# facebookresearch/fast3r

Hardware: NVIDIA H100
Metric: views_per_sec (higher is better)
Workload: dtype bf16

## Files before the change

fast3r_b200/csrc/capi.cu:

```cuda
#include <cstdarg>
#include <cstdio>
#include <cstdlib>
#include <cstring>

#include "../../include/fast3r_b200.h"
#include "f3r_kernels.h"
#include "gemm_plan.h"

namespace {

thread_local char g_err[512] = "";

int fail(const char* fmt, ...) {
  va_list ap;
  va_start(ap, fmt);
  vsnprintf(g_err, sizeof(g_err), fmt, ap);
  va_end(ap);
  return 1;
}
int check(cudaError_t e, const char* what) {
  if (e == cudaSuccess) return 0;
  return fail("%s: %s", what, cudaGetErrorString(e));
}

// ... 68 lines not shown
  if (d->k % 8 || d->a_ld % 8) return fail("f3r_gemm: k=%d and a_ld=%d must be multiples of 8", d->k, d->a_ld);
  if (d->taps != 1 && d->taps != 9) return fail("f3r_gemm: taps must be 1 or 9");
  if (d->epi == F3R_EPI_FINAL && d->n != 128) return fail("f3r_gemm: FINAL epilogue needs n == 128");
  if (d->epi == F3R_EPI_CONVT && (d->ct_k <= 0 || d->ct_cout % 32 || d->n != d->ct_k * d->ct_k * d->ct_cout))
    return fail("f3r_gemm: bad CONVT geometry");
  if (d->epi == F3R_EPI_ROPE && (!d->rope_cos || !d->rope_sin || d->tok_per_img <= 0 || d->grid_w <= 0))
    return fail("f3r_gemm: bad ROPE arguments");
  if (d->epi == F3R_EPI_IDXEMB && (!d->emb_table || !d->emb_ids || d->tok_per_img < 0))
    return fail("f3r_gemm: bad IDXEMB arguments");
  if (d->f16 != 0 && d->f16 != 1) return fail("f3r_gemm: f16=%d must be 0 or 1", d->f16);

  static int dbg = -1, tma_pref = -1, ksplit_pref = -1;
  if (dbg < 0) { const char* e = getenv("F3R_GEMM_DEBUG"); dbg = e ? atoi(e) : 0; }
  if (tma_pref < 0) { const char* e = getenv("F3R_GEMM_TMA_EPI"); tma_pref = (e && e[0] == '0') ? 0 : 1; }
  if (ksplit_pref < 0) { const char* e = getenv("F3R_GEMM_KSPLIT"); ksplit_pref = (e && e[0] == '1') ? 1 : 0; }
  const f3r::GemmPlan plan = f3r::gemm_plan(*d, num_sms(), tma_pref, ksplit_pref != 1);
  const int block_n = plan.block_n;

  f3r::GemmArgs a;
  memset(&a, 0, sizeof(a));
  a.M = d->w * d->h * d->nb; a.N = d->n; a.K = d->k; a.taps = d->taps;
  a.W = d->w; a.H = d->h; a.NB = d->nb;
  a.bw = plan.bw; a.bh = plan.bh; a.bw_log2 = plan.bw_log2; a.sbx_log2 = plan.sbx_log2;
  a.tiles_x = plan.tiles_x; a.tiles_y = plan.tiles_y; a.num_m_tiles = plan.num_m_tiles;
  a.num_n_tiles = plan.num_n_tiles;
  a.tma_epi = plan.tma_epi; a.k_split = plan.k_split;
  a.debug = dbg;
  a.epi = d->epi; a.act = d->act; a.out0_f32 = d->out0_f32; a.res0_f32 = d->res0_f32;
  a.ldo = d->ldo > 0 ? d->ldo : d->n;
  a.split_col = d->split_col; a.ldo_b = d->ldo_b;
  a.tok_per_img = d->tok_per_img; a.grid_w = d->grid_w; a.rope_cols = d->rope_cols;
  a.ct_k = d->ct_k; a.ct_cout = d->ct_cout;
  a.bias = d->bias; a.res0 = d->res0; a.res1 = d->res1;
  a.out0 = d->out0; a.out0b = d->out0b; a.out1 = d->out1;
  a.rope_cos = d->rope_cos; a.rope_sin = d->rope_sin;
  a.emb_table = d->emb_table; a.emb_ids = d->emb_ids;
  a.w4 = d->w4; a.b4 = d->b4; a.pts = d->pts; a.conf = d->conf;
  if (a.split_col && (a.split_col % 32 || !a.out0b)) return fail("f3r_gemm: bad column split");

  const CUtensorMapDataType t16 = d->f16 ? CU_TENSOR_MAP_DATA_TYPE_FLOAT16 : CU_TENSOR_MAP_DATA_TYPE_BFLOAT16;
  CUtensorMap ta, tb;
  {
    const uint64_t ld = static_cast<uint64_t>(d->a_ld) * 2;
    const uint64_t dims[4] = {static_cast<uint64_t>(d->k), static_cast<uint64_t>(d->w),
                              static_cast<uint64_t>(d->h), static_cast<uint64_t>(d->nb)};
    const uint64_t str[3] = {ld, ld * d->w, ld * d->w * d->h};
    const uint32_t box[4] = {64, static_cast<uint32_t>(a.bw), static_cast<uint32_t>(a.bh), 1};
    if (make_tmap(&ta, d->a, 4, dims, str, box, t16)) return 1;
  }
  {
    const uint64_t dims[3] = {static_cast<uint64_t>(d->k), static_cast<uint64_t>(d->taps),
                              static_cast<uint64_t>(d->n)};
    const uint64_t str[2] = {static_cast<uint64_t>(d->k) * 2, static_cast<uint64_t>(d->k) * 2 * d->taps};
    const uint32_t box[3] = {64, 1, static_cast<uint32_t>(block_n)};
    if (make_tmap(&tb, d->wt, 3, dims, str, box, t16)) return 1;
  }
  CUtensorMap to0, to0b;
  memset(&to0, 0, sizeof(to0));
  memset(&to0b, 0, sizeof(to0b));
  if (a.tma_epi) {
    const uint64_t es = d->out0_f32 ? 4 : 2;
    const CUtensorMapDataType dt = d->out0_f32 ? CU_TENSOR_MAP_DATA_TYPE_FLOAT32 : t16;
    const CUtensorMapSwizzle sw = d->out0_f32 ? CU_TENSOR_MAP_SWIZZLE_128B : CU_TENSOR_MAP_SWIZZLE_64B;
    const uint32_t sbx = 1u << a.sbx_log2;
    const uint32_t box[4] = {32, sbx, 32 / sbx, 1};
    const uint64_t ncols0 = a.split_col ? a.split_col : d->n;
    {
      const uint64_t ld = static_cast<uint64_t>(a.ldo) * es;
      const uint64_t dims[4] = {ncols0, static_cast<uint64_t>(d->w), static_cast<uint64_t>(d->h),
                                static_cast<uint64_t>(d->nb)};
      const uint64_t str[3] = {ld, ld * d->w, ld * d->w * d->h};
      if (make_tmap(&to0, d->out0, 4, dims, str, box, dt, sw)) return 1;
    }
    if (a.split_col) {
      const uint64_t ld = static_cast<uint64_t>(a.ldo_b) * es;
      const uint64_t dims[4] = {static_cast<uint64_t>(d->n - a.split_col), static_cast<uint64_t>(d->w),
                                static_cast<uint64_t>(d->h), static_cast<uint64_t>(d->nb)};
      const uint64_t str[3] = {ld, ld * d->w, ld * d->w * d->h};
      if (make_tmap(&to0b, d->out0b, 4, dims, str, box, dt, sw)) return 1;
    }
  }
  return check(f3r::launch_gemm(block_n, d->f16, ta, tb, to0, to0b, a, num_sms(), static_cast<cudaStream_t>(stream)),
               "f3r_gemm");
}

static int attention_impl(const char* what, int f16, const void* q, int32_t ldq, const void* kv, int32_t ldkv,
                          int32_t kv_rows_total, int32_t kv_row0, void* out, int32_t ldo, float* lse, float* part_o,
                          float* part_lse, int32_t part_base, int32_t n_split, int32_t batch, int32_t heads, int32_t sq,
                          int32_t skv, float scale, void* stream) {
  const CUtensorMapDataType t16 = f16 ? CU_TENSOR_MAP_DATA_TYPE_FLOAT16 : CU_TENSOR_MAP_DATA_TYPE_BFLOAT16;
  if (!q || !kv) return fail("%s: null operand", what);
  if (batch <= 0 || heads <= 0 || sq <= 0 || skv <= 0) return fail("%s: bad shape", what);
  if (ldq % 8 || ldkv % 8 || ldq < heads * 64 || ldkv < 2 * heads * 64) return fail("%s: bad leading dimensions", what);
  if (kv_row0 < 0 || kv_row0 + skv > kv_rows_total) return fail("%s: key range outside the kv buffer", what);
  if (n_split < 1 || n_split > (skv + 127) / 128) return fail("%s: n_split=%d must be in [1, #key blocks]", what, n_split);
  CUtensorMap tq, tkv;
  {
    const uint64_t dims[3] = {static_cast<uint64_t>(heads) * 64, static_cast<uint64_t>(sq),
                              static_cast<uint64_t>(batch)};
    const uint64_t str[2] = {static_cast<uint64_t>(ldq) * 2, static_cast<uint64_t>(ldq) * 2 * sq};
    const uint32_t box[3] = {64, f3r::ATT_Q_TILE, 1};
    if (make_tmap(&tq, q, 3, dims, str, box, t16)) return 1;
  }
  {
    const uint64_t dims[3] = {static_cast<uint64_t>(heads) * 128, static_cast<uint64_t>(kv_row0 + skv),
                              static_cast<uint64_t>(batch)};
    const uint64_t str[2] = {static_cast<uint64_t>(ldkv) * 2, static_cast<uint64_t>(ldkv) * 2 * kv_rows_total};
// ... 549 lines not shown
```

fast3r_b200/csrc/common.cuh:

```cuda
#pragma once
#include <cuda.h>
#include <cuda_bf16.h>
#include <cuda_fp16.h>
#include <cuda_runtime.h>
#include <stdint.h>

#include <type_traits>

namespace f3r {

#define F3R_DEVICE __device__ __forceinline__

F3R_DEVICE uint32_t smem_u32(const void* p) { return static_cast<uint32_t>(__cvta_generic_to_shared(p)); }

F3R_DEVICE uint32_t lane_id() { return threadIdx.x & 31; }

F3R_DEVICE bool elect_one() {
  uint32_t pred = 0;
  asm volatile(
      "{\n\t.reg .pred P;\n\t"
      "elect.sync _|P, 0xffffffff;\n\t"
      "selp.u32 %0, 1, 0, P;\n\t}\n"
      : "=r"(pred));
  return pred != 0;
// ... 16 lines not shown
  asm volatile(
      "{\n\t.reg .pred P;\n\t"
      "mbarrier.try_wait.parity.shared::cta.b64 P, [%1], %2;\n\t"
      "selp.u32 %0, 1, 0, P;\n\t}\n"
      : "=r"(ok)
      : "r"(smem_u32(bar)), "r"(parity)
      : "memory");
  return ok != 0;
}
F3R_DEVICE void mbar_wait(uint64_t* bar, uint32_t parity) {
  while (!mbar_try_wait(bar, parity)) {
  }
}

F3R_DEVICE void mbar_wait_relaxed(uint64_t* bar, uint32_t parity) {
  while (!mbar_try_wait(bar, parity)) asm volatile("nanosleep.u32 64;");
}

F3R_DEVICE void tma_prefetch_desc(const CUtensorMap* m) {
  asm volatile("prefetch.tensormap [%0];" ::"l"(reinterpret_cast<uint64_t>(m)) : "memory");
}
F3R_DEVICE void tma_load_2d(void* dst, const CUtensorMap* m, uint64_t* bar, int c0, int c1) {
  asm volatile(
      "cp.async.bulk.tensor.2d.shared::cluster.global.mbarrier::complete_tx::bytes [%0], [%1, {%3, %4}], [%2];"
      ::"r"(smem_u32(dst)), "l"(reinterpret_cast<uint64_t>(m)), "r"(smem_u32(bar)), "r"(c0), "r"(c1)
      : "memory");
}
F3R_DEVICE void tma_load_3d(void* dst, const CUtensorMap* m, uint64_t* bar, int c0, int c1, int c2) {
  asm volatile(
      "cp.async.bulk.tensor.3d.shared::cluster.global.mbarrier::complete_tx::bytes [%0], [%1, {%3, %4, %5}], [%2];"
      ::"r"(smem_u32(dst)), "l"(reinterpret_cast<uint64_t>(m)), "r"(smem_u32(bar)), "r"(c0), "r"(c1), "r"(c2)
      : "memory");
}
F3R_DEVICE void tma_load_4d(void* dst, const CUtensorMap* m, uint64_t* bar, int c0, int c1, int c2, int c3) {
  asm volatile(
      "cp.async.bulk.tensor.4d.shared::cluster.global.mbarrier::complete_tx::bytes [%0], [%1, {%3, %4, %5, %6}], [%2];"
      ::"r"(smem_u32(dst)), "l"(reinterpret_cast<uint64_t>(m)), "r"(smem_u32(bar)), "r"(c0), "r"(c1), "r"(c2),
      "r"(c3)
      : "memory");
}

F3R_DEVICE void tma_store_4d(const CUtensorMap* m, const void* src, int c0, int c1, int c2, int c3) {
  asm volatile("cp.async.bulk.tensor.4d.global.shared::cta.bulk_group [%0, {%2, %3, %4, %5}], [%1];"
               ::"l"(reinterpret_cast<uint64_t>(m)), "r"(smem_u32(src)), "r"(c0), "r"(c1), "r"(c2), "r"(c3)
               : "memory");
}
F3R_DEVICE void tma_reduce_add_4d(const CUtensorMap* m, const void* src, int c0, int c1, int c2, int c3) {
  asm volatile("cp.reduce.async.bulk.tensor.4d.global.shared::cta.add.tile.bulk_group [%0, {%2, %3, %4, %5}], [%1];"
               ::"l"(reinterpret_cast<uint64_t>(m)), "r"(smem_u32(src)), "r"(c0), "r"(c1), "r"(c2), "r"(c3)
               : "memory");
}
F3R_DEVICE void tma_store_commit() { asm volatile("cp.async.bulk.commit_group;" ::: "memory"); }
F3R_DEVICE void tma_store_wait_read() { asm volatile("cp.async.bulk.wait_group.read 0;" ::: "memory"); }
F3R_DEVICE void tma_store_wait_all() { asm volatile("cp.async.bulk.wait_group 0;" ::: "memory"); }

F3R_DEVICE void pdl_wait() { asm volatile("griddepcontrol.wait;" ::: "memory"); }
F3R_DEVICE void pdl_launch_dependents() { asm volatile("griddepcontrol.launch_dependents;" ::: "memory"); }

F3R_DEVICE uint32_t cluster_ctarank() { uint32_t r; asm volatile("mov.u32 %0, %%cluster_ctarank;" : "=r"(r)); return r; }
F3R_DEVICE uint32_t cluster_id_x() { uint32_t r; asm volatile("mov.u32 %0, %%clusterid.x;" : "=r"(r)); return r; }
F3R_DEVICE uint32_t num_clusters_x() { uint32_t r; asm volatile("mov.u32 %0, %%nclusterid.x;" : "=r"(r)); return r; }
F3R_DEVICE void cluster_sync_all() {
  asm volatile("barrier.cluster.arrive.release.aligned;" ::: "memory");
  asm volatile("barrier.cluster.wait.acquire.aligned;" ::: "memory");
}

F3R_DEVICE uint64_t make_smem_desc_sw128(uint32_t smem_addr) {
  uint64_t d = 0;
  d |= static_cast<uint64_t>((smem_addr & 0x3FFFF) >> 4);
  d |= static_cast<uint64_t>(1) << 16;
  d |= static_cast<uint64_t>(1024 >> 4) << 32;
  d |= static_cast<uint64_t>(1) << 62;
  return d;
}
F3R_DEVICE void wgmma_fence() { asm volatile("wgmma.fence.sync.aligned;" ::: "memory"); }
F3R_DEVICE void wgmma_commit() { asm volatile("wgmma.commit_group.sync.aligned;" ::: "memory"); }
template <int kPending>
F3R_DEVICE void wgmma_wait() { asm volatile("wgmma.wait_group.sync.aligned %0;" ::"n"(kPending) : "memory"); }
template <int kN>
F3R_DEVICE void fence_regs(float (&d)[kN]) {
#pragma unroll
  for (int i = 0; i < kN; ++i) asm volatile("" : "+f"(d[i])::"memory");
}


template <typename T>
constexpr bool is_f16 = std::is_same<T, __half>::value;

#define F3R_WGMMA_SS_N128(TY) \
  asm volatile( \
      "{\n\t.reg .pred p;\n\t" \
      "setp.ne.b32 p, %66, 0;\n\t" \
      "wgmma.mma_async.sync.aligned.m64n128k16.f32." TY "." TY " {%0, %1, %2, %3, %4, %5, %6, %7, %8, %9, %10, %11, %12, %13, %14, %15, %16, %17, %18, %19, %20, %21, %22, %23, %24, %25, %26, %27, %28, %29, %30, %31, %32, %33, %34, %35, %36, %37, %38, %39, %40, %41, %42, %43, %44, %45, %46, %47, %48, %49, %50, %51, %52, %53, %54, %55, %56, %57, %58, %59, %60, %61, %62, %63}, %64, %65, p, 1, 1, 0, %67;\n\t}\n" \
      : "+f"(d[0]), "+f"(d[1]), "+f"(d[2]), "+f"(d[3]), "+f"(d[4]), "+f"(d[5]), "+f"(d[6]), "+f"(d[7]), "+f"(d[8]), "+f"(d[9]), "+f"(d[10]), "+f"(d[11]), "+f"(d[12]), "+f"(d[13]), "+f"(d[14]), "+f"(d[15]), "+f"(d[16]), "+f"(d[17]), "+f"(d[18]), "+f"(d[19]), "+f"(d[20]), "+f"(d[21]), "+f"(d[22]), "+f"(d[23]), "+f"(d[24]), "+f"(d[25]), "+f"(d[26]), "+f"(d[27]), "+f"(d[28]), "+f"(d[29]), "+f"(d[30]), "+f"(d[31]), "+f"(d[32]), "+f"(d[33]), "+f"(d[34]), "+f"(d[35]), "+f"(d[36]), "+f"(d[37]), "+f"(d[38]), "+f"(d[39]), "+f"(d[40]), "+f"(d[41]), "+f"(d[42]), "+f"(d[43]), "+f"(d[44]), "+f"(d[45]), "+f"(d[46]), "+f"(d[47]), "+f"(d[48]), "+f"(d[49]), "+f"(d[50]), "+f"(d[51]), "+f"(d[52]), "+f"(d[53]), "+f"(d[54]), "+f"(d[55]), "+f"(d[56]), "+f"(d[57]), "+f"(d[58]), "+f"(d[59]), "+f"(d[60]), "+f"(d[61]), "+f"(d[62]), "+f"(d[63]) \
      : "l"(a_desc), "l"(b_desc), "r"(accumulate), "n"(kTransB))
template <int kTransB, typename T = __nv_bfloat16>
F3R_DEVICE void wgmma_ss_n128(float (&d)[64], uint64_t a_desc, uint64_t b_desc, uint32_t accumulate) {
  if constexpr (is_f16<T>) F3R_WGMMA_SS_N128("f16");
  else F3R_WGMMA_SS_N128("bf16");
}

#define F3R_WGMMA_SS_N256(TY) \
  asm volatile( \
      "{\n\t.reg .pred p;\n\t" \
      "setp.ne.b32 p, %130, 0;\n\t" \
      "wgmma.mma_async.sync.aligned.m64n256k16.f32." TY "." TY " {%0, %1, %2, %3, %4, %5, %6, %7, %8, %9, %10, %11, %12, %13, %14, %15, %16, %17, %18, %19, %20, %21, %22, %23, %24, %25, %26, %27, %28, %29, %30, %31, %32, %33, %34, %35, %36, %37, %38, %39, %40, %41, %42, %43, %44, %45, %46, %47, %48, %49, %50, %51, %52, %53, %54, %55, %56, %57, %58, %59, %60, %61, %62, %63, %64, %65, %66, %67, %68, %69, %70, %71, %72, %73, %74, %75, %76, %77, %78, %79, %80, %81, %82, %83, %84, %85, %86, %87, %88, %89, %90, %91, %92, %93, %94, %95, %96, %97, %98, %99, %100, %101, %102, %103, %104, %105, %106, %107, %108, %109, %110, %111, %112, %113, %114, %115, %116, %117, %118, %119, %120, %121, %122, %123, %124, %125, %126, %127}, %128, %129, p, 1, 1, 0, %131;\n\t}\n" \
// ... 50 lines not shown
```

fast3r_b200/csrc/gemm.cu:

```cuda
#include "common.cuh"
#include "f3r_kernels.h"

namespace f3r {

constexpr int BLOCK_M = 128;
constexpr int BLOCK_K = 64;
constexpr int GEMM_THREADS = 384;
constexpr int XCH_STRIDE = 68;

template <int BLOCK_N>
struct GemmCfg {
  static constexpr int kStages = (BLOCK_N == 256) ? 3 : 4;
  static constexpr int kABytes = BLOCK_M * BLOCK_K * 2;
  static constexpr int kBBytes = BLOCK_N * BLOCK_K * 2;
  static constexpr int kStageBytes = kABytes + kBBytes;
  static constexpr int kXchBytes = 64 * XCH_STRIDE * 4;
  static constexpr int kSmemBytes =
      kStages * kStageBytes + 1024  + 1024  + 8 * 4096  + 2 * kXchBytes;
};

struct ResChunk {
  uint4 r0[8];
  uint2 r1[8];
};

__device__ __forceinline__ size_t out_offset(const GemmArgs& p, int m, int col0, int img, int py, int px) {
  if (p.epi == EPI_CONVT) {
    const int ij = col0 / p.ct_cout, o0 = col0 % p.ct_cout, k = p.ct_k;
    const int oy = py * k + ij / k, ox = px * k + ij % k;
    return ((static_cast<size_t>(img) * p.H * k + oy) * (p.W * k) + ox) * p.ct_cout + o0;
  }
  return static_cast<size_t>(m) * p.ldo + col0;
}

__device__ __forceinline__ void prefetch_res(const GemmArgs& p, ResChunk& rc, size_t off_row, bool ok_row, int lane) {
  if (p.res0 == nullptr && p.res1 == nullptr) return;
  const unsigned okmask = __ballot_sync(0xffffffffu, ok_row);
#pragma unroll
  for (int i = 0; i < 8; ++i) {
    const int rr = 4 * i + (lane >> 3);
    const size_t off = __shfl_sync(0xffffffffu, off_row, rr) + (lane & 7) * 4;
    if (!((okmask >> rr) & 1)) continue;
    if (p.res0 != nullptr) {
      if (p.res0_f32) rc.r0[i] = *reinterpret_cast<const uint4*>(static_cast<const float*>(p.res0) + off);
      else {
        const uint2 t = *reinterpret_cast<const uint2*>(static_cast<const uint16_t*>(p.res0) + off);
        rc.r0[i].x = t.x; rc.r0[i].y = t.y;
      }
    }
    if (p.res1 != nullptr) rc.r1[i] = *reinterpret_cast<const uint2*>(static_cast<const uint16_t*>(p.res1) + off);
  }
}

__device__ __forceinline__ void gelu_fast(float& x) {
  const float z = __fmul_rn(fabsf(x), 0.70710678118654752440f);
  const float u = fmaf(z, 0.3275911f, 1.0f);
  float t;
  asm("rcp.approx.ftz.f32 %0, %1;" : "=f"(t) : "f"(u));
  float q = fmaf(t, 1.061405429f, -1.453152027f);
  q = fmaf(q, t, 1.421413741f);
  q = fmaf(q, t, -0.284496736f);
  q = fmaf(q, t, 0.254829592f);
  q = __fmul_rn(q, t);
  const float a = __fmul_rn(__fmul_rn(z, z), -1.4426950408889634f);
  float e;
  asm("ex2.approx.ftz.f32 %0, %1;" : "=f"(e) : "f"(a));
  const float r = copysignf(fmaf(q, -e, 1.0f), x);
// ... 10 lines not shown
      v[4 * i + 0] += b.x; v[4 * i + 1] += b.y; v[4 * i + 2] += b.z; v[4 * i + 3] += b.w;
    }
  }
  if (p.epi == EPI_ROPE && col0 < p.rope_cols && row_ok) {
    const int t = m % p.tok_per_img;
    const int pos = ((col0 >> 5) & 1) ? (t % p.grid_w) : (t / p.grid_w);
    const float4* c4 = reinterpret_cast<const float4*>(p.rope_cos + pos * 16);
    const float4* s4 = reinterpret_cast<const float4*>(p.rope_sin + pos * 16);
#pragma unroll
    for (int i = 0; i < 4; ++i) {
      float4 c = __ldg(c4 + i), s = __ldg(s4 + i);
      float cc[4] = {c.x, c.y, c.z, c.w}, ss[4] = {s.x, s.y, s.z, s.w};
#pragma unroll
      for (int e = 0; e < 4; ++e) {
        const int j = 4 * i + e;
        const float a = v[j], b = v[j + 16];
        v[j] = a * cc[e] - b * ss[e];
        v[j + 16] = b * cc[e] + a * ss[e];
      }
    }
  }
  if (p.epi == EPI_IDXEMB && row_ok) {
    const int id = __ldg(p.emb_ids + (p.tok_per_img > 0 ? m / p.tok_per_img : m));
    const float4* e4 = reinterpret_cast<const float4*>(p.emb_table + static_cast<size_t>(id) * p.N + col0);
#pragma unroll
    for (int i = 0; i < 8; ++i) {
      float4 e = __ldg(e4 + i);
      v[4 * i + 0] += e.x; v[4 * i + 1] += e.y; v[4 * i + 2] += e.z; v[4 * i + 3] += e.w;
    }
  }
  if (p.epi == EPI_FINAL) {
    if (row_ok) {
#pragma unroll
      for (int o = 0; o < 4; ++o) {
        const float4* w = reinterpret_cast<const float4*>(w4s + o * p.N + col0);
        float acc = fin[o];
#pragma unroll
        for (int i = 0; i < 8; ++i) {
          const float4 ww = w[i];
          acc = fmaf(fmaxf(v[4 * i + 0], 0.f), ww.x, acc);
          acc = fmaf(fmaxf(v[4 * i + 1], 0.f), ww.y, acc);
          acc = fmaf(fmaxf(v[4 * i + 2], 0.f), ww.z, acc);
          acc = fmaf(fmaxf(v[4 * i + 3], 0.f), ww.w, acc);
        }
        fin[o] = acc;
      }
    }
    return false;
  }
  return true;
}

template <typename T>
__device__ __forceinline__ void epilogue_store(const GemmArgs& p, const float (&v)[32], const ResChunk& rc, uint8_t* stage,
                                               int lane, int m, int col0, size_t off_row, bool ok_row) {
  using H = Half16<T>;
#pragma unroll
  for (int j = 0; j < 8; ++j)
    *reinterpret_cast<float4*>(stage + lane * 128 + ((j ^ (lane & 7)) << 4)) =
        make_float4(v[4 * j], v[4 * j + 1], v[4 * j + 2], v[4 * j + 3]);
  __syncwarp();
  const unsigned okmask = __ballot_sync(0xffffffffu, ok_row);
  const int cj = lane & 7;
  const bool to_b = p.split_col > 0 && col0 >= p.split_col;
#pragma unroll
  for (int i = 0; i < 8; ++i) {
    const int rr = 4 * i + (lane >> 3);
    const size_t off = __shfl_sync(0xffffffffu, off_row, rr) + cj * 4;
    const int mrow = __shfl_sync(0xffffffffu, m, rr);
    if (!((okmask >> rr) & 1)) continue;
    const float4 a = *reinterpret_cast<const float4*>(stage + rr * 128 + ((cj ^ (rr & 7)) << 4));
    float x0 = a.x, x1 = a.y, x2 = a.z, x3 = a.w;
    if (p.res0 != nullptr) {
      if (p.res0_f32) {
        x0 += __uint_as_float(rc.r0[i].x); x1 += __uint_as_float(rc.r0[i].y);
        x2 += __uint_as_float(rc.r0[i].z); x3 += __uint_as_float(rc.r0[i].w);
      } else {
        x0 += H::lo(rc.r0[i].x); x1 += H::hi(rc.r0[i].x); x2 += H::lo(rc.r0[i].y); x3 += H::hi(rc.r0[i].y);
      }
    }
    if (p.res1 != nullptr) {
      x0 += H::lo(rc.r1[i].x); x1 += H::hi(rc.r1[i].x); x2 += H::lo(rc.r1[i].y); x3 += H::hi(rc.r1[i].y);
    }
    if (p.out1 != nullptr) {
      uint2 o;
      o.x = H::pack(fmaxf(x0, 0.f), fmaxf(x1, 0.f));
      o.y = H::pack(fmaxf(x2, 0.f), fmaxf(x3, 0.f));
      *reinterpret_cast<uint2*>(static_cast<T*>(p.out1) + off) = o;
    }
    if (p.out0 == nullptr) continue;
    if (p.act == ACT_RELU) {
      x0 = fmaxf(x0, 0.f); x1 = fmaxf(x1, 0.f); x2 = fmaxf(x2, 0.f); x3 = fmaxf(x3, 0.f);
    } else if (p.act == ACT_GELU) {
      gelu_fast(x0); gelu_fast(x1); gelu_fast(x2); gelu_fast(x3);
    }
    void* base = p.out0;
    size_t o = off;
    if (to_b) {
      base = p.out0b;
      o = static_cast<size_t>(mrow) * p.ldo_b + (col0 - p.split_col) + cj * 4;
    }
    if (p.out0_f32) {
      *reinterpret_cast<float4*>(static_cast<float*>(base) + o) = make_float4(x0, x1, x2, x3);
    } else {
      uint2 q;
      q.x = H::pack(x0, x1);
      q.y = H::pack(x2, x3);
      *reinterpret_cast<uint2*>(static_cast<T*>(base) + o) = q;
    }
  }
  __syncwarp();
}

template <typename T>
__device__ __forceinline__ void epilogue_tma(const GemmArgs& p, float (&v)[32], uint8_t* stage, int lane,
                                             const CUtensorMap* map, bool reduce, int c_col, int c_x, int c_y, int c_img) {
  if (p.act == ACT_RELU) {
#pragma unroll
    for (int i = 0; i < 32; ++i) v[i] = fmaxf(v[i], 0.f);
  } else if (p.act == ACT_GELU) {
#pragma unroll
    for (int i = 0; i < 32; ++i) gelu_fast(v[i]);
  }
  if (lane == 0) tma_store_wait_read();
  __syncwarp();
  if (p.out0_f32) {
#pragma unroll
    for (int j = 0; j < 8; ++j)
      *reinterpret_cast<float4*>(stage + lane * 128 + ((j ^ (lane & 7)) << 4)) =
          make_float4(v[4 * j], v[4 * j + 1], v[4 * j + 2], v[4 * j + 3]);
  } else {
#pragma unroll
    for (int j = 0; j < 4; ++j) {
      uint4 q;
      q.x = Half16<T>::pack(v[8 * j + 0], v[8 * j + 1]);
      q.y = Half16<T>::pack(v[8 * j + 2], v[8 * j + 3]);
      q.z = Half16<T>::pack(v[8 * j + 4], v[8 * j + 5]);
      q.w = Half16<T>::pack(v[8 * j + 6], v[8 * j + 7]);
      *reinterpret_cast<uint4*>(stage + lane * 64 + ((j ^ ((lane >> 1) & 3)) << 4)) = q;
    }
  }
  fence_proxy_async_smem();
  __syncwarp();
  if (lane == 0) {
    if (reduce) tma_reduce_add_4d(map, stage, c_col, c_x, c_y, c_img);
    else tma_store_4d(map, stage, c_col, c_x, c_y, c_img);
    tma_store_commit();
  }
}

template <int BLOCK_N, typename T>
__global__ void __launch_bounds__(GEMM_THREADS, 1)
gemm_kernel(const __grid_constant__ CUtensorMap tmap_a, const __grid_constant__ CUtensorMap tmap_b,
            const __grid_constant__ CUtensorMap tmap_o0, const __grid_constant__ CUtensorMap tmap_o0b,
            const __grid_constant__ GemmArgs p) {
  using Cfg = GemmCfg<BLOCK_N>;
  extern __shared__ uint8_t smem_raw[];
  uint8_t* smem = reinterpret_cast<uint8_t*>((reinterpret_cast<uintptr_t>(smem_raw) + 1023) & ~uintptr_t(1023));
  uint8_t* smem_a = smem;
  uint8_t* smem_b = smem + Cfg::kStages * Cfg::kABytes;
  uint64_t* bars = reinterpret_cast<uint64_t*>(smem + Cfg::kStages * Cfg::kStageBytes);
  uint64_t* full_bar = bars;
  uint64_t* empty_bar = bars + Cfg::kStages;
  uint8_t* stage_base = smem + Cfg::kStages * Cfg::kStageBytes + 1024;
  float* fin_smem = reinterpret_cast<float*>(stage_base);
  float* w4_smem = reinterpret_cast<float*>(stage_base + 4096);
  float* xch_base = reinterpret_cast<float*>(stage_base + 8 * 4096);

  const int warp = threadIdx.x >> 5;
  const int lane = threadIdx.x & 31;

  if (threadIdx.x == 0) {
    tma_prefetch_desc(&tmap_a);
    tma_prefetch_desc(&tmap_b);
    for (int s = 0; s < Cfg::kStages; ++s) { mbar_init(&full_bar[s], 1); mbar_init(&empty_bar[s], 2); }
    fence_barrier_init();
  }
  if (p.epi == EPI_FINAL)
    for (int i = threadIdx.x; i < 4 * p.N; i += GEMM_THREADS) w4_smem[i] = __ldg(p.w4 + i);
  __syncthreads();
  pdl_wait();
  pdl_launch_dependents();

  const int num_out_tiles = p.num_m_tiles * p.num_n_tiles;
  const int num_tiles = num_out_tiles * p.k_split;
  const int k_chunks = (p.K + BLOCK_K - 1) / BLOCK_K;
  const int k_iters = p.taps * k_chunks;

  if (warp < 4) {
    asm volatile("setmaxnreg.dec.sync.aligned.u32 40;");
    if (warp == 0 && lane == 0) {
      int stage = 0; uint32_t phase = 0;
      for (int item = blockIdx.x; item < num_tiles; item += gridDim.x) {
        const int tile = item % num_out_tiles, ks = item / num_out_tiles;
        const int it0 = ks * k_iters / p.k_split, it1 = (ks + 1) * k_iters / p.k_split;
        const int mt = tile / p.num_n_tiles, nt = tile % p.num_n_tiles;
        const int tx = mt % p.tiles_x, ty = (mt / p.tiles_x) % p.tiles_y, img = mt / (p.tiles_x * p.tiles_y);
        const int x0 = tx * p.bw, y0 = ty * p.bh, n0 = nt * BLOCK_N;
        for (int it = it0; it < it1; ++it) {
          const int tap = it / k_chunks, kc = it % k_chunks;
          int dy = 0, dx = 0;
          if (p.taps == 9) { dy = tap / 3 - 1; dx = tap % 3 - 1; }
          mbar_wait_relaxed(&empty_bar[stage], phase ^ 1);
          mbar_arrive_expect_tx(&full_bar[stage], Cfg::kStageBytes);
          tma_load_4d(smem_a + stage * Cfg::kABytes, &tmap_a, &full_bar[stage], kc * BLOCK_K, x0 + dx, y0 + dy, img);
          tma_load_3d(smem_b + stage * Cfg::kBBytes, &tmap_b, &full_bar[stage], kc * BLOCK_K, tap, n0);
          if (++stage == Cfg::kStages) { stage = 0; phase ^= 1; }
        }
      }
    }
  } else {
    asm volatile("setmaxnreg.inc.sync.aligned.u32 232;");
    const int cg = (warp - 4) >> 2;
    const int wg_warp = warp & 3;
    const int wg_tid = threadIdx.x & 127;
    const int half = wg_warp >> 1;
    const int r_loc = (wg_warp & 1) * 32 + lane;
    const int r = cg * 64 + r_loc;
    float* xch = xch_base + cg * 64 * XCH_STRIDE;
    uint8_t* stage_buf = stage_base + (warp - 4) * 4096;
    const int bar_id = 1 + cg;
    constexpr int kAcc = BLOCK_N / 2;
    int stage = 0; uint32_t phase = 0;
    for (int item = blockIdx.x; item < num_tiles; item += gridDim.x) {
      const int tile = item % num_out_tiles, ks = item / num_out_tiles;
      const int it0 = ks * k_iters / p.k_split, it1 = (ks + 1) * k_iters / p.k_split;
      const bool add_bias = ks == 0;
      float acc[kAcc];
#pragma unroll
      for (int i = 0; i < kAcc; ++i) acc[i] = 0.f;
      int prev = -1;
      for (int it = it0; it < it1; ++it) {
        mbar_wait(&full_bar[stage], phase);
        const uint64_t a_desc = make_smem_desc_sw128(smem_u32(smem_a + stage * Cfg::kABytes + cg * 64 * 128));
        const uint64_t b_desc = make_smem_desc_sw128(smem_u32(smem_b + stage * Cfg::kBBytes));
        fence_regs(acc);
        wgmma_fence();
#pragma unroll
        for (int k = 0; k < BLOCK_K / 16; ++k) {
          if constexpr (BLOCK_N == 256) wgmma_ss_n256<0, T>(acc, a_desc + 2 * k, b_desc + 2 * k, 1u);
          else wgmma_ss_n128<0, T>(acc, a_desc + 2 * k, b_desc + 2 * k, 1u);
        }
        wgmma_commit();
        wgmma_wait<1>();
        fence_regs(acc);
        if (prev >= 0 && wg_tid == 0) mbar_arrive(&empty_bar[prev]);
        prev = stage;
        if (++stage == Cfg::kStages) { stage = 0; phase ^= 1; }
      }
      wgmma_wait<0>();
      fence_regs(acc);
      if (prev >= 0 && wg_tid == 0) mbar_arrive(&empty_bar[prev]);

      const int mt = tile / p.num_n_tiles, nt = tile % p.num_n_tiles;
      const int tx = mt % p.tiles_x, ty = (mt / p.tiles_x) % p.tiles_y, img = mt / (p.tiles_x * p.tiles_y);
      const int px = tx * p.bw + r % p.bw, py = ty * p.bh + r / p.bw;
      const bool row_ok = (px < p.W) && (py < p.H) && (mt < p.num_m_tiles);
      const int m = (img * p.H + py) * p.W + px;
      const int n_valid = min(BLOCK_N / 32, (p.N - nt * BLOCK_N + 31) / 32);
      float fin[4] = {0.f, 0.f, 0.f, 0.f};
#pragma unroll
      for (int cp = 0; cp < BLOCK_N / 64; ++cp) {
        asm volatile("bar.sync %0, 128;" ::"r"(bar_id) : "memory");
        {
          const int fr = wg_warp * 16 + (lane >> 2), fc = 2 * (lane & 3);
#pragma unroll
          for (int j = 0; j < 8; ++j) {
            const int jj = cp * 8 + j;
            *reinterpret_cast<float2*>(xch + fr * XCH_STRIDE + 8 * j + fc) = make_float2(acc[4 * jj], acc[4 * jj + 1]);
            *reinterpret_cast<float2*>(xch + (fr + 8) * XCH_STRIDE + 8 * j + fc) =
                make_float2(acc[4 * jj + 2], acc[4 * jj + 3]);
          }
        }
        asm volatile("bar.sync %0, 128;" ::"r"(bar_id) : "memory");
        const int c = 2 * cp + half;
        if (c >= n_valid) continue;
        const int col0 = nt * BLOCK_N + c * 32;
        float v[32];
#pragma unroll
        for (int i = 0; i < 8; ++i) {
          const float4 t = *reinterpret_cast<const float4*>(xch + r_loc * XCH_STRIDE + half * 32 + 4 * i);
          v[4 * i] = t.x; v[4 * i + 1] = t.y; v[4 * i + 2] = t.z; v[4 * i + 3] = t.w;
        }
        if (epilogue_rows(p, v, m, col0, row_ok, fin, add_bias, w4_smem) && !(p.debug & 1)) {
          if (p.tma_epi) {
            const bool to_b = p.split_col > 0 && col0 >= p.split_col;
            const int r0 = cg * 64 + (wg_warp & 1) * 32;
            epilogue_tma<T>(p, v, stage_buf, lane, to_b ? &tmap_o0b : &tmap_o0, p.tma_epi == 2,
                         to_b ? col0 - p.split_col : col0, tx * p.bw + (r0 & (p.bw - 1)), ty * p.bh + (r0 >> p.bw_log2),
                         mt < p.num_m_tiles ? img : p.NB);
          } else {
            const size_t off = out_offset(p, m, col0, img, py, px);
            ResChunk rc;
            prefetch_res(p, rc, off, row_ok, lane);
            epilogue_store<T>(p, v, rc, stage_buf, lane, m, col0, off, row_ok);
          }
        }
      }
      if (p.epi == EPI_FINAL) {
        float* slot = fin_smem + r * 4;
        if (half == 1) { slot[0] = fin[0]; slot[1] = fin[1]; slot[2] = fin[2]; slot[3] = fin[3]; }
        asm volatile("bar.sync %0, 128;" ::"r"(bar_id) : "memory");
        if (half == 0 && row_ok) {
          const float x = fin[0] + slot[0] + __ldg(p.b4 + 0), y = fin[1] + slot[1] + __ldg(p.b4 + 1);
          const float z = fin[2] + slot[2] + __ldg(p.b4 + 2), c = fin[3] + slot[3] + __ldg(p.b4 + 3);
          const float d = sqrtf(x * x + y * y + z * z);
          const float sc = expm1f(d) / fmaxf(d, 1e-8f);
          float* pt = p.pts + static_cast<size_t>(m) * 3;
          pt[0] = x * sc; pt[1] = y * sc; pt[2] = z * sc;
          p.conf[m] = 1.f + expf(c);
        }
      }
    }
    if (p.tma_epi && lane == 0) tma_store_wait_all();
  }
}

template <int BLOCK_N, typename T>
static cudaError_t launch_gemm_t(const CUtensorMap& ta, const CUtensorMap& tb, const CUtensorMap& to0,
                                 const CUtensorMap& to0b, const GemmArgs& a, int num_sms, cudaStream_t stream) {
  const int items = a.num_m_tiles * a.num_n_tiles * a.k_split;
  return launch(gemm_kernel<BLOCK_N, T>, items < num_sms ? items : num_sms, GEMM_THREADS, GemmCfg<BLOCK_N>::kSmemBytes,
                stream, true, ta, tb, to0, to0b, a);
}

cudaError_t launch_gemm(int block_n, int f16, const CUtensorMap& ta, const CUtensorMap& tb, const CUtensorMap& to0,
                        const CUtensorMap& to0b, const GemmArgs& a, int num_sms, cudaStream_t stream) {
  if (f16) {
    if (block_n == 256) return launch_gemm_t<256, __half>(ta, tb, to0, to0b, a, num_sms, stream);
    return launch_gemm_t<128, __half>(ta, tb, to0, to0b, a, num_sms, stream);
  }
  if (block_n == 256) return launch_gemm_t<256, __nv_bfloat16>(ta, tb, to0, to0b, a, num_sms, stream);
  return launch_gemm_t<128, __nv_bfloat16>(ta, tb, to0, to0b, a, num_sms, stream);
}

}
```

Measured before the change: 151.9.

## Add ping-pong consumer schedule with 128-wide N sub-tiles in persistent GEMM

Restructures the warp-specialized GEMM so each consumer warpgroup computes a full 128x128 sub-tile (two M-halves) and the two warpgroups alternate sub-tiles via named ordering barriers, letting one warpgroup's epilogue overlap the other's MMA mainloop. BLOCK_N=256 tiles are split into two 128-column sub-tiles with a fixed 4-stage ring, and the cooperative path is kept for split-K or small grids. Also double-buffers TMA epilogue staging (wait for all but one pending store) and moves residual prefetch into the store routine. This raises register pressure (two 64-float accumulators per thread) and adds barrier complexity in exchange for hiding epilogue latency.

```diff
diff --git a/fast3r_b200/csrc/capi.cu b/fast3r_b200/csrc/capi.cu
--- a/fast3r_b200/csrc/capi.cu
+++ b/fast3r_b200/csrc/capi.cu
@@ -144,7 +144,7 @@
     const uint64_t dims[3] = {static_cast<uint64_t>(d->k), static_cast<uint64_t>(d->taps),
                               static_cast<uint64_t>(d->n)};
     const uint64_t str[2] = {static_cast<uint64_t>(d->k) * 2, static_cast<uint64_t>(d->k) * 2 * d->taps};
-    const uint32_t box[3] = {64, 1, static_cast<uint32_t>(block_n)};
+    const uint32_t box[3] = {64, 1, 128};
     if (make_tmap(&tb, d->wt, 3, dims, str, box, t16)) return 1;
   }
   CUtensorMap to0, to0b;
diff --git a/fast3r_b200/csrc/common.cuh b/fast3r_b200/csrc/common.cuh
--- a/fast3r_b200/csrc/common.cuh
+++ b/fast3r_b200/csrc/common.cuh
@@ -92,6 +92,7 @@
 }
 F3R_DEVICE void tma_store_commit() { asm volatile("cp.async.bulk.commit_group;" ::: "memory"); }
 F3R_DEVICE void tma_store_wait_read() { asm volatile("cp.async.bulk.wait_group.read 0;" ::: "memory"); }
+F3R_DEVICE void tma_store_wait_read_but1() { asm volatile("cp.async.bulk.wait_group.read 1;" ::: "memory"); }
 F3R_DEVICE void tma_store_wait_all() { asm volatile("cp.async.bulk.wait_group 0;" ::: "memory"); }
 
 F3R_DEVICE void pdl_wait() { asm volatile("griddepcontrol.wait;" ::: "memory"); }
diff --git a/fast3r_b200/csrc/gemm.cu b/fast3r_b200/csrc/gemm.cu
--- a/fast3r_b200/csrc/gemm.cu
+++ b/fast3r_b200/csrc/gemm.cu
@@ -8,11 +8,13 @@
 constexpr int GEMM_THREADS = 384;
 constexpr int XCH_STRIDE = 68;
 
-template <int BLOCK_N>
+constexpr int SUB_N = 128;
+constexpr int ORDER_BAR = 3;
+
 struct GemmCfg {
-  static constexpr int kStages = (BLOCK_N == 256) ? 3 : 4;
+  static constexpr int kStages = 4;
   static constexpr int kABytes = BLOCK_M * BLOCK_K * 2;
-  static constexpr int kBBytes = BLOCK_N * BLOCK_K * 2;
+  static constexpr int kBBytes = SUB_N * BLOCK_K * 2;
   static constexpr int kStageBytes = kABytes + kBBytes;
   static constexpr int kXchBytes = 64 * XCH_STRIDE * 4;
   static constexpr int kSmemBytes =
@@ -129,13 +131,15 @@
 }
 
 template <typename T>
-__device__ __forceinline__ void epilogue_store(const GemmArgs& p, const float (&v)[32], const ResChunk& rc, uint8_t* stage,
-                                               int lane, int m, int col0, size_t off_row, bool ok_row) {
+__device__ __forceinline__ void epilogue_store(const GemmArgs& p, const float (&v)[32], uint8_t* stage, int lane, int m,
+                                               int col0, size_t off_row, bool ok_row) {
   using H = Half16<T>;
 #pragma unroll
   for (int j = 0; j < 8; ++j)
     *reinterpret_cast<float4*>(stage + lane * 128 + ((j ^ (lane & 7)) << 4)) =
         make_float4(v[4 * j], v[4 * j + 1], v[4 * j + 2], v[4 * j + 3]);
+  ResChunk rc;
+  prefetch_res(p, rc, off_row, ok_row, lane);
   __syncwarp();
   const unsigned okmask = __ballot_sync(0xffffffffu, ok_row);
   const int cj = lane & 7;
@@ -190,8 +194,9 @@
 }
 
 template <typename T>
-__device__ __forceinline__ void epilogue_tma(const GemmArgs& p, float (&v)[32], uint8_t* stage, int lane,
-                                             const CUtensorMap* map, bool reduce, int c_col, int c_x, int c_y, int c_img) {
+__device__ __forceinline__ void epilogue_tma(const GemmArgs& p, float (&v)[32], uint8_t* stage_tile, bool upper,
+                                             bool wait_all, int lane, const CUtensorMap* map, bool reduce, int c_col,
+                                             int c_x, int c_y, int c_img) {
   if (p.act == ACT_RELU) {
 #pragma unroll
     for (int i = 0; i < 32; ++i) v[i] = fmaxf(v[i], 0.f);
@@ -199,7 +204,13 @@
 #pragma unroll
     for (int i = 0; i < 32; ++i) gelu_fast(v[i]);
   }
-  if (lane == 0) tma_store_wait_read();
+  uint8_t* stage = stage_tile;
+  if (p.out0_f32 || wait_all) {
+    if (lane == 0) tma_store_wait_read();
+  } else {
+    if (lane == 0) tma_store_wait_read_but1();
+  }
+  if (!p.out0_f32 && upper) stage += 2048;
   __syncwarp();
   if (p.out0_f32) {
 #pragma unroll
@@ -226,12 +237,19 @@
   }
 }
 
-template <int BLOCK_N, typename T>
+__device__ __forceinline__ void ring_advance(int& stage, uint32_t& phase, int n) {
+  const int t = stage + n;
+  phase ^= static_cast<uint32_t>(t / GemmCfg::kStages) & 1u;
+  stage = t % GemmCfg::kStages;
+}
+
+template <int BLOCK_N, typename T, bool COOP>
 __global__ void __launch_bounds__(GEMM_THREADS, 1)
 gemm_kernel(const __grid_constant__ CUtensorMap tmap_a, const __grid_constant__ CUtensorMap tmap_b,
             const __grid_constant__ CUtensorMap tmap_o0, const __grid_constant__ CUtensorMap tmap_o0b,
             const __grid_constant__ GemmArgs p) {
-  using Cfg = GemmCfg<BLOCK_N>;
+  using Cfg = GemmCfg;
+  constexpr int kSubs = BLOCK_N / SUB_N;
   extern __shared__ uint8_t smem_raw[];
   uint8_t* smem = reinterpret_cast<uint8_t*>((reinterpret_cast<uintptr_t>(smem_raw) + 1023) & ~uintptr_t(1023));
   uint8_t* smem_a = smem;
@@ -247,10 +265,16 @@
   const int warp = threadIdx.x >> 5;
   const int lane = threadIdx.x & 31;
 
+  const int num_out_tiles = p.num_m_tiles * p.num_n_tiles;
+  const int num_tiles = num_out_tiles * p.k_split;
+  const int k_chunks = (p.K + BLOCK_K - 1) / BLOCK_K;
+  const int k_iters = p.taps * k_chunks;
+  constexpr bool coop = COOP;
+
   if (threadIdx.x == 0) {
     tma_prefetch_desc(&tmap_a);
     tma_prefetch_desc(&tmap_b);
-    for (int s = 0; s < Cfg::kStages; ++s) { mbar_init(&full_bar[s], 1); mbar_init(&empty_bar[s], 2); }
+    for (int s = 0; s < Cfg::kStages; ++s) { mbar_init(&full_bar[s], 1); mbar_init(&empty_bar[s], coop ? 2 : 1); }
     fence_barrier_init();
   }
   if (p.epi == EPI_FINAL)
@@ -258,11 +282,6 @@
   __syncthreads();
   pdl_wait();
   pdl_launch_dependents();
-
-  const int num_out_tiles = p.num_m_tiles * p.num_n_tiles;
-  const int num_tiles = num_out_tiles * p.k_split;
-  const int k_chunks = (p.K + BLOCK_K - 1) / BLOCK_K;
-  const int k_iters = p.taps * k_chunks;
 
   if (warp < 4) {
     asm volatile("setmaxnreg.dec.sync.aligned.u32 40;");
@@ -273,16 +292,19 @@
         const int it0 = ks * k_iters / p.k_split, it1 = (ks + 1) * k_iters / p.k_split;
         const int mt = tile / p.num_n_tiles, nt = tile % p.num_n_tiles;
         const int tx = mt % p.tiles_x, ty = (mt / p.tiles_x) % p.tiles_y, img = mt / (p.tiles_x * p.tiles_y);
-        const int x0 = tx * p.bw, y0 = ty * p.bh, n0 = nt * BLOCK_N;
-        for (int it = it0; it < it1; ++it) {
-          const int tap = it / k_chunks, kc = it % k_chunks;
-          int dy = 0, dx = 0;
-          if (p.taps == 9) { dy = tap / 3 - 1; dx = tap % 3 - 1; }
-          mbar_wait_relaxed(&empty_bar[stage], phase ^ 1);
-          mbar_arrive_expect_tx(&full_bar[stage], Cfg::kStageBytes);
-          tma_load_4d(smem_a + stage * Cfg::kABytes, &tmap_a, &full_bar[stage], kc * BLOCK_K, x0 + dx, y0 + dy, img);
-          tma_load_3d(smem_b + stage * Cfg::kBBytes, &tmap_b, &full_bar[stage], kc * BLOCK_K, tap, n0);
-          if (++stage == Cfg::kStages) { stage = 0; phase ^= 1; }
+        const int x0 = tx * p.bw, y0 = ty * p.bh;
+        for (int s = 0; s < kSubs; ++s) {
+          const int n0 = nt * BLOCK_N + s * SUB_N;
+          for (int it = it0; it < it1; ++it) {
+            const int tap = it / k_chunks, kc = it % k_chunks;
+            int dy = 0, dx = 0;
+            if (p.taps == 9) { dy = tap / 3 - 1; dx = tap % 3 - 1; }
+            mbar_wait_relaxed(&empty_bar[stage], phase ^ 1);
+            mbar_arrive_expect_tx(&full_bar[stage], Cfg::kStageBytes);
+            tma_load_4d(smem_a + stage * Cfg::kABytes, &tmap_a, &full_bar[stage], kc * BLOCK_K, x0 + dx, y0 + dy, img);
+            tma_load_3d(smem_b + stage * Cfg::kBBytes, &tmap_b, &full_bar[stage], kc * BLOCK_K, tap, n0);
+            ring_advance(stage, phase, 1);
+          }
         }
       }
     }
@@ -293,101 +315,129 @@
     const int wg_tid = threadIdx.x & 127;
     const int half = wg_warp >> 1;
     const int r_loc = (wg_warp & 1) * 32 + lane;
-    const int r = cg * 64 + r_loc;
     float* xch = xch_base + cg * 64 * XCH_STRIDE;
     uint8_t* stage_buf = stage_base + (warp - 4) * 4096;
     const int bar_id = 1 + cg;
-    constexpr int kAcc = BLOCK_N / 2;
+    if (cg == 1 && !coop) asm volatile("bar.arrive %0, 256;" ::"r"(ORDER_BAR) : "memory");
+    auto sub_iters = [&](int jj) {
+      const int ks = (blockIdx.x + (jj / kSubs) * gridDim.x) / num_out_tiles;
+      return (ks + 1) * k_iters / p.k_split - ks * k_iters / p.k_split;
+    };
     int stage = 0; uint32_t phase = 0;
-    for (int item = blockIdx.x; item < num_tiles; item += gridDim.x) {
+    for (int j = coop ? 0 : cg;; j += coop ? 1 : 2) {
+      const int u = j / kSubs, s = j % kSubs;
+      const int item = blockIdx.x + u * gridDim.x;
+      if (item >= num_tiles) break;
+      if (j > 0 && !coop) ring_advance(stage, phase, sub_iters(j - 1));
       const int tile = item % num_out_tiles, ks = item / num_out_tiles;
       const int it0 = ks * k_iters / p.k_split, it1 = (ks + 1) * k_iters / p.k_split;
       const bool add_bias = ks == 0;
-      float acc[kAcc];
-#pragma unroll
-      for (int i = 0; i < kAcc; ++i) acc[i] = 0.f;
+      const bool last = blockIdx.x + ((j + 1) / kSubs) * gridDim.x >= num_tiles;
+      const int mt = tile / p.num_n_tiles, nt = tile % p.num_n_tiles;
+      const int n0 = nt * BLOCK_N + s * SUB_N;
+      const int tx = mt % p.tiles_x, ty = (mt / p.tiles_x) % p.tiles_y, img = mt / (p.tiles_x * p.tiles_y);
+      float acc[2][64];
+#pragma unroll
+      for (int i = 0; i < 64; ++i) { acc[0][i] = 0.f; acc[1][i] = 0.f; }
+      if (!coop) asm volatile("bar.sync %0, 256;" ::"r"(ORDER_BAR + cg) : "memory");
       int prev = -1;
       for (int it = it0; it < it1; ++it) {
         mbar_wait(&full_bar[stage], phase);
-        const uint64_t a_desc = make_smem_desc_sw128(smem_u32(smem_a + stage * Cfg::kABytes + cg * 64 * 128));
+        const uint32_t a_addr = smem_u32(smem_a + stage * Cfg::kABytes);
+        const uint64_t a_desc0 = make_smem_desc_sw128(a_addr + (coop ? cg * 64 * 128 : 0));
+        const uint64_t a_desc1 = make_smem_desc_sw128(a_addr + 64 * 128);
         const uint64_t b_desc = make_smem_desc_sw128(smem_u32(smem_b + stage * Cfg::kBBytes));
-        fence_regs(acc);
+        fence_regs(acc[0]);
+        fence_regs(acc[1]);
         wgmma_fence();
-#pragma unroll
-        for (int k = 0; k < BLOCK_K / 16; ++k) {
-          if constexpr (BLOCK_N == 256) wgmma_ss_n256<0, T>(acc, a_desc + 2 * k, b_desc + 2 * k, 1u);
-          else wgmma_ss_n128<0, T>(acc, a_desc + 2 * k, b_desc + 2 * k, 1u);
+        if (coop) {
+#pragma unroll
+          for (int k = 0; k < BLOCK_K / 16; ++k) wgmma_ss_n128<0, T>(acc[0], a_desc0 + 2 * k, b_desc + 2 * k, 1u);
+        } else {
+#pragma unroll
+          for (int k = 0; k < BLOCK_K / 16; ++k) {
+            wgmma_ss_n128<0, T>(acc[0], a_desc0 + 2 * k, b_desc + 2 * k, 1u);
+            wgmma_ss_n128<0, T>(acc[1], a_desc1 + 2 * k, b_desc + 2 * k, 1u);
+          }
         }
         wgmma_commit();
         wgmma_wait<1>();
-        fence_regs(acc);
+        fence_regs(acc[0]);
+        fence_regs(acc[1]);
         if (prev >= 0 && wg_tid == 0) mbar_arrive(&empty_bar[prev]);
         prev = stage;
-        if (++stage == Cfg::kStages) { stage = 0; phase ^= 1; }
-      }
+        ring_advance(stage, phase, 1);
+      }
+      if (!last && !coop) asm volatile("bar.arrive %0, 256;" ::"r"(ORDER_BAR + (cg ^ 1)) : "memory");
       wgmma_wait<0>();
-      fence_regs(acc);
+      fence_regs(acc[0]);
+      fence_regs(acc[1]);
       if (prev >= 0 && wg_tid == 0) mbar_arrive(&empty_bar[prev]);
 
-      const int mt = tile / p.num_n_tiles, nt = tile % p.num_n_tiles;
-      const int tx = mt % p.tiles_x, ty = (mt / p.tiles_x) % p.tiles_y, img = mt / (p.tiles_x * p.tiles_y);
-      const int px = tx * p.bw + r % p.bw, py = ty * p.bh + r / p.bw;
-      const bool row_ok = (px < p.W) && (py < p.H) && (mt < p.num_m_tiles);
-      const int m = (img * p.H + py) * p.W + px;
-      const int n_valid = min(BLOCK_N / 32, (p.N - nt * BLOCK_N + 31) / 32);
-      float fin[4] = {0.f, 0.f, 0.f, 0.f};
-#pragma unroll
-      for (int cp = 0; cp < BLOCK_N / 64; ++cp) {
-        asm volatile("bar.sync %0, 128;" ::"r"(bar_id) : "memory");
-        {
-          const int fr = wg_warp * 16 + (lane >> 2), fc = 2 * (lane & 3);
-#pragma unroll
-          for (int j = 0; j < 8; ++j) {
-            const int jj = cp * 8 + j;
-            *reinterpret_cast<float2*>(xch + fr * XCH_STRIDE + 8 * j + fc) = make_float2(acc[4 * jj], acc[4 * jj + 1]);
-            *reinterpret_cast<float2*>(xch + (fr + 8) * XCH_STRIDE + 8 * j + fc) =
-                make_float2(acc[4 * jj + 2], acc[4 * jj + 3]);
+      const int n_valid = min(SUB_N / 32, (p.N - n0 + 31) / 32);
+#pragma unroll
+      for (int h = 0; h < 2; ++h) {
+        if (coop && h == 1) break;
+        const int hr = coop ? cg : h;
+        const int r = hr * 64 + r_loc;
+        const int px = tx * p.bw + r % p.bw, py = ty * p.bh + r / p.bw;
+        const bool row_ok = (px < p.W) && (py < p.H) && (mt < p.num_m_tiles);
+        const int m = (img * p.H + py) * p.W + px;
+        float fin[4] = {0.f, 0.f, 0.f, 0.f};
+#pragma unroll
+        for (int cp = 0; cp < SUB_N / 64; ++cp) {
+          asm volatile("bar.sync %0, 128;" ::"r"(bar_id) : "memory");
+          {
+            const int fr = wg_warp * 16 + (lane >> 2), fc = 2 * (lane & 3);
+#pragma unroll
+            for (int jf = 0; jf < 8; ++jf) {
+              const int jj = cp * 8 + jf;
+              *reinterpret_cast<float2*>(xch + fr * XCH_STRIDE + 8 * jf + fc) =
+                  make_float2(acc[h][4 * jj], acc[h][4 * jj + 1]);
+              *reinterpret_cast<float2*>(xch + (fr + 8) * XCH_STRIDE + 8 * jf + fc) =
+                  make_float2(acc[h][4 * jj + 2], acc[h][4 * jj + 3]);
+            }
+          }
+          asm volatile("bar.sync %0, 128;" ::"r"(bar_id) : "memory");
+          const int c = 2 * cp + half;
+          if (c >= n_valid) continue;
+          const int col0 = n0 + c * 32;
+          float v[32];
+#pragma unroll
+          for (int i = 0; i < 8; ++i) {
+            const float4 t = *reinterpret_cast<const float4*>(xch + r_loc * XCH_STRIDE + half * 32 + 4 * i);
+            v[4 * i] = t.x; v[4 * i + 1] = t.y; v[4 * i + 2] = t.z; v[4 * i + 3] = t.w;
+          }
+          if (epilogue_rows(p, v, m, col0, row_ok, fin, add_bias, w4_smem) && !(p.debug & 1)) {
+            if (p.tma_epi) {
+              const bool to_b = p.split_col > 0 && col0 >= p.split_col;
+              const int r0 = hr * 64 + (wg_warp & 1) * 32;
+              epilogue_tma<T>(p, v, stage_buf, cp == 1, cp == 0 && n_valid < SUB_N / 32, lane,
+                           to_b ? &tmap_o0b : &tmap_o0, p.tma_epi == 2,
+                           to_b ? col0 - p.split_col : col0, tx * p.bw + (r0 & (p.bw - 1)),
+                           ty * p.bh + (r0 >> p.bw_log2), mt < p.num_m_tiles ? img : p.NB);
+            } else {
+              const size_t off = out_offset(p, m, col0, img, py, px);
+              epilogue_store<T>(p, v, stage_buf, lane, m, col0, off, row_ok);
+            }
           }
         }
-        asm volatile("bar.sync %0, 128;" ::"r"(bar_id) : "memory");
-        const int c = 2 * cp + half;
-        if (c >= n_valid) continue;
-        const int col0 = nt * BLOCK_N + c * 32;
-        float v[32];
-#pragma unroll
-        for (int i = 0; i < 8; ++i) {
-          const float4 t = *reinterpret_cast<const float4*>(xch + r_loc * XCH_STRIDE + half * 32 + 4 * i);
-          v[4 * i] = t.x; v[4 * i + 1] = t.y; v[4 * i + 2] = t.z; v[4 * i + 3] = t.w;
+        if (p.epi == EPI_FINAL) {
+          float* slot = fin_smem + (cg * 64 + r_loc) * 4;
+          if (half == 1) { slot[0] = fin[0]; slot[1] = fin[1]; slot[2] = fin[2]; slot[3] = fin[3]; }
+          asm volatile("bar.sync %0, 128;" ::"r"(bar_id) : "memory");
+          if (half == 0 && row_ok) {
+            const float x = fin[0] + slot[0] + __ldg(p.b4 + 0), y = fin[1] + slot[1] + __ldg(p.b4 + 1);
+            const float z = fin[2] + slot[2] + __ldg(p.b4 + 2), c = fin[3] + slot[3] + __ldg(p.b4 + 3);
+            const float d = sqrtf(x * x + y * y + z * z);
+            const float sc = expm1f(d) / fmaxf(d, 1e-8f);
+            float* pt = p.pts + static_cast<size_t>(m) * 3;
+            pt[0] = x * sc; pt[1] = y * sc; pt[2] = z * sc;
+            p.conf[m] = 1.f + expf(c);
+          }
         }
-        if (epilogue_rows(p, v, m, col0, row_ok, fin, add_bias, w4_smem) && !(p.debug & 1)) {
-          if (p.tma_epi) {
-            const bool to_b = p.split_col > 0 && col0 >= p.split_col;
-            const int r0 = cg * 64 + (wg_warp & 1) * 32;
-            epilogue_tma<T>(p, v, stage_buf, lane, to_b ? &tmap_o0b : &tmap_o0, p.tma_epi == 2,
-                         to_b ? col0 - p.split_col : col0, tx * p.bw + (r0 & (p.bw - 1)), ty * p.bh + (r0 >> p.bw_log2),
-                         mt < p.num_m_tiles ? img : p.NB);
-          } else {
-            const size_t off = out_offset(p, m, col0, img, py, px);
-            ResChunk rc;
-            prefetch_res(p, rc, off, row_ok, lane);
-            epilogue_store<T>(p, v, rc, stage_buf, lane, m, col0, off, row_ok);
-          }
-        }
-      }
-      if (p.epi == EPI_FINAL) {
-        float* slot = fin_smem + r * 4;
-        if (half == 1) { slot[0] = fin[0]; slot[1] = fin[1]; slot[2] = fin[2]; slot[3] = fin[3]; }
-        asm volatile("bar.sync %0, 128;" ::"r"(bar_id) : "memory");
-        if (half == 0 && row_ok) {
-          const float x = fin[0] + slot[0] + __ldg(p.b4 + 0), y = fin[1] + slot[1] + __ldg(p.b4 + 1);
-          const float z = fin[2] + slot[2] + __ldg(p.b4 + 2), c = fin[3] + slot[3] + __ldg(p.b4 + 3);
-          const float d = sqrtf(x * x + y * y + z * z);
-          const float sc = expm1f(d) / fmaxf(d, 1e-8f);
-          float* pt = p.pts + static_cast<size_t>(m) * 3;
-          pt[0] = x * sc; pt[1] = y * sc; pt[2] = z * sc;
-          p.conf[m] = 1.f + expf(c);
-        }
-      }
+      }
+      if (p.tma_epi && n_valid < SUB_N / 32 && lane == 0) tma_store_wait_read();
     }
     if (p.tma_epi && lane == 0) tma_store_wait_all();
   }
@@ -397,8 +447,12 @@
 static cudaError_t launch_gemm_t(const CUtensorMap& ta, const CUtensorMap& tb, const CUtensorMap& to0,
                                  const CUtensorMap& to0b, const GemmArgs& a, int num_sms, cudaStream_t stream) {
   const int items = a.num_m_tiles * a.num_n_tiles * a.k_split;
-  return launch(gemm_kernel<BLOCK_N, T>, items < num_sms ? items : num_sms, GEMM_THREADS, GemmCfg<BLOCK_N>::kSmemBytes,
-                stream, true, ta, tb, to0, to0b, a);
+  const int grid = items < num_sms ? items : num_sms;
+  if (a.k_split > 1 || (BLOCK_N == 128 && items <= num_sms))
+    return launch(gemm_kernel<BLOCK_N, T, true>, grid, GEMM_THREADS, GemmCfg::kSmemBytes, stream, true, ta, tb, to0,
+                  to0b, a);
+  return launch(gemm_kernel<BLOCK_N, T, false>, grid, GEMM_THREADS, GemmCfg::kSmemBytes, stream, true, ta, tb, to0,
+                to0b, a);
 }
 
 cudaError_t launch_gemm(int block_n, int f16, const CUtensorMap& ta, const CUtensorMap& tb, const CUtensorMap& to0,
```

Result: faster. 153.6, median of 6 (+1.1%).
